# zhengyk19/vit-rpe-rope

Measured on AMD Instinct MI355X. Metric: train images/sec, CIFAR-10 ViT d=192 L=6 H=6, higher is better.
Workload: dtype bf16; 1 GPU; CIFAR-10-shaped 32x32 patch4 ViT d=192 L=6 H=6, --pos_encoding rope-axial theta=100, bf16, full train step (fwd+CE+bwd+AdamW), random-init weights; per_gpu_batch=512, global_batch=512, parallelism=dp1, hip_graph=True

## Files before the change

### include/vitpe_debug.h

```cpp
#ifndef VITPE_DEBUG_H
#define VITPE_DEBUG_H
#include "vitpe.h"
#ifdef __cplusplus
extern "C" {
#endif

int vitpe_selftest_mma(int dtype, const void* A, const void* Bt, const void* Brow, float* C_row,
                       float* C_tr, vitpe_stream_t stream);

int vitpe_debug_attn_occupancy(int which);
int vitpe_debug_wgrad_census(int dtype, const vitpe_wgrad_problem* problems, int nprob, unsigned long long* census,
                             vitpe_stream_t stream);
int vitpe_debug_attn_census(const void* xn, const void* wqkv, void* out, const float* cos, const float* sin,
                            int B, unsigned long long* census, vitpe_stream_t stream);
int vitpe_debug_attn32_census(const void* xn, const void* wqkv_wide, void* out, const float* cos, const float* sin,
                              int B, unsigned long long* census, int exp, vitpe_stream_t stream);
int vitpe_debug_tail2_census(const void* attn_out, const void* x_in, const void* Wp_packed, const float* bp,
                             const float* gamma, const float* beta, void* x_mid, float* mean2, float* rstd2,
                             void* xn_out, const void* W1_packed, const float* b1, const void* W2_packed,
                             const float* b2, void* gp_out, void* h_out, void* out, float* mean_out, float* rstd_out,
                             int M, int HID, unsigned long long* census, int exp, vitpe_stream_t stream);
int vitpe_debug_set_gemm2d_mt(int mt);
int vitpe_debug_set_wgrad_wide(int on);
int vitpe_debug_read_bw(const void* src, long long bytes, int depth, int workgroups, unsigned* sink, vitpe_stream_t stream);
#ifdef __cplusplus
}
#endif
#endif
```

### vit-rpe-rope_amd/csrc/attn.hip

```cpp
#include "attn_common.h"
#include <stdlib.h>
#include <type_traits>

namespace vitpe {

template <typename T, typename C, int KM, int NTH = 384>
VITPE_DEV void stage_tokens(const AttnArgs& a, int b, T* xs, T* hbuf, int hbuf_elems, float* s_tab, float* s_coef,
                            int tid, int nthreads, bool stage_tables) {
  constexpr int CHN = CH<T>::n;
  constexpr int DCH = C::LDX / CHN;
  constexpr int D = C::DD;
  const int N = C::ntok(a);
  const T* xg = reinterpret_cast<const T*>(a.xn) + (size_t)b * N * D;
  const Chunk16 zero = {0u, 0u, 0u, 0u};
  constexpr int TOTAL = C::NP * DCH;
  constexpr int ITERS = (TOTAL + NTH - 1) / NTH;
  Chunk16 v[ITERS];
#pragma unroll
  for (int it = 0; it < ITERS; ++it) {
    const int q = tid + it * nthreads, row = q / DCH, cc = q % DCH;
    v[it] = zero;
    if (q < TOTAL && row < N && cc * CHN < D) v[it] = *reinterpret_cast<const Chunk16*>(xg + (size_t)row * D + cc * CHN);
  }
  if (a.ln_gamma != nullptr) {
// ... 340 lines not shown
    f32x4 o[NT];
#pragma unroll
    for (int dt = 0; dt < NT; ++dt) o[dt] = z4;
#pragma unroll
    for (int sc = 0; sc < SC; ++sc) {
      const Frag<T> bp = acc_to_frag<T>(s[2 * sc], (2 * sc + 1 < MT) ? s[(2 * sc + 1 < MT) ? 2 * sc + 1 : 0] : z4);
#pragma unroll
      for (int dt = 0; dt < NT; ++dt) mma(vf[dt][sc], bp, o[dt]);
    }
    const float inv = __builtin_amdgcn_rcpf(l);
    if (sizeof(T) == 2) {
#pragma unroll
      for (int dp = 0; dp < NT; dp += 2) {
        uint32_t lo[2], hi[2];
#pragma unroll
        for (int w2 = 0; w2 < 2; ++w2) {
          bf16x2 pa, pb;
          const f32x4 oa = o[dp] * inv, ob = o[dp + 1] * inv;
          pa[0] = (bf16)oa[2 * w2]; pa[1] = (bf16)oa[2 * w2 + 1];
          pb[0] = (bf16)ob[2 * w2]; pb[1] = (bf16)ob[2 * w2 + 1];
          const auto r = __builtin_amdgcn_permlane16_swap(__builtin_bit_cast(uint32_t, pa), __builtin_bit_cast(uint32_t, pb),
                                                         false, false);
          lo[w2] = r[0]; hi[w2] = r[1];
        }
        const int f0 = 16 * (dp + (g & 1)) + 8 * (g >> 1);
        if (it < MT - 1 || i < N)
          *reinterpret_cast<Chunk16*>(outp + (size_t)i * D + f0) = (Chunk16){lo[0], lo[1], hi[0], hi[1]};
      }
    } else if (it < MT - 1 || i < N) {
#pragma unroll
      for (int dt = 0; dt < NT; ++dt)
        st4(outp + (size_t)i * D + 16 * dt + 4 * g, o[dt][0] * inv, o[dt][1] * inv, o[dt][2] * inv, o[dt][3] * inv);
    }
  }
  stamp(6);
}

template <typename T, typename C, int NTH>
VITPE_DEV void stage_rows_plain(const T* src, T* dst, int ld, int N, int tid) {
  constexpr int CHN = CH<T>::n, D = C::DD, CPRW = D / CHN, RPP = NTH / CPRW, ITERS = C::NP / RPP;
  const int cc = tid % CPRW, r0 = tid / CPRW;
  const Chunk16 zero = {0u, 0u, 0u, 0u};
  Chunk16 v[ITERS];
#pragma unroll
  for (int it = 0; it < ITERS; ++it) {
    const int row = r0 + it * RPP;
    v[it] = *reinterpret_cast<const Chunk16*>(src + (size_t)min(row, N - 1) * D + cc * CHN);
    if (row >= N) v[it] = zero;
  }
#pragma unroll
  for (int it = 0; it < ITERS; ++it) *reinterpret_cast<Chunk16*>(dst + (r0 + it * RPP) * ld + cc * CHN) = v[it];
}

template <int HD, int D, int MT, int KM, int NTOK, int IPW, bool LNF, bool MIXED, int PDEG = 7>
__global__ __launch_bounds__(64 * (D / HD) * IPW, 3) void attn_bwd_reg_kernel(AttnArgs a) {
  using T = bf16;
  using C = AttnCfg<T, HD, D, MT, 1, NTOK>;
  constexpr int NT = C::NT, KS = C::KS, HC = C::HC, SC = C::SC, NTH = 64 * C::H;
  static_assert(NT == 2 && HC == 1, "head dimension 32");
  constexpr int CSLD = HD / 2 + 8;
  constexpr int FRAG = 64 * 8;
  constexpr int XS_ELEMS = IPW * C::NP * C::LDX, DOS_ELEMS = IPW * C::H * MT * FRAG;
  __shared__ __attribute__((aligned(16))) T xs_all[XS_ELEMS > DOS_ELEMS ? XS_ELEMS : DOS_ELEMS];
  __shared__ __attribute__((aligned(16))) T qs_all[IPW * C::H * MT * FRAG];
  __shared__ __attribute__((aligned(16))) float s_tab[KM == KM_RELATIVE ? C::H * C::TABLD : 4];
  __shared__ __attribute__((aligned(16))) float s_coef[KM == KM_POLY ? C::PESZ : 4];
  __shared__ __attribute__((aligned(16))) float s_cos[KM == KM_ROPE ? C::NP * CSLD : 4];
  __shared__ __attribute__((aligned(16))) float s_sin[KM == KM_ROPE ? C::NP * CSLD : 4];
  __shared__ __attribute__((aligned(16))) float s_stat[IPW * C::H * 2 * C::NP];
  __shared__ float s_dtab[KM == KM_RELATIVE ? C::H * C::TABLD : 4];
  __shared__ float s_dcoef[C::H * (C::MAXDEG + 1)];
  __shared__ float s_dfreq[2 * C::H * (HD / 2)];

  const int N = C::ntok(a), P = N - 1;
  const int lane = threadIdx.x & 63;
  const int wave_all = __builtin_amdgcn_readfirstlane(threadIdx.x >> 6);
  const int img = wave_all / C::H, h = wave_all % C::H;
  const int b_raw = blockIdx.x * IPW + img;
  const bool live = b_raw < a.B;
  const int b = live ? b_raw : a.B - 1;
  const int tid_img = threadIdx.x % NTH;
  T* const xs = xs_all + img * C::NP * C::LDX;
  T* const qsw = qs_all + wave_all * MT * FRAG + lane * 8;
  T* const dsw = xs_all + wave_all * MT * FRAG + lane * 8;
  float* const lse_w = s_stat + (img * C::H + h) * 2 * C::NP;
  float* const del_w = lse_w + C::NP;
  float* const dtab_i = s_dtab;
  float* const dcoef_i = s_dcoef;
  float* const dfreq_i = s_dfreq;
  const int c = lane & 15, g = lane >> 4;
  const f32x4 z4 = {0.f, 0.f, 0.f, 0.f};
  constexpr bool mixed = (KM == KM_ROPE) && MIXED;

  const T* const Wh = reinterpret_cast<const T*>(a.wqkv) + ((size_t)h * 3 * NT * KS * 64 + lane) * 8;
  auto wload = [&](Frag<T> (&w)[NT][KS], int mat) {
#pragma unroll
    for (int nt = 0; nt < NT; ++nt)
#pragma unroll
      for (int ks = 0; ks < KS; ++ks) w[nt][ks] = ld_frag(Wh + (size_t)((mat * NT + nt) * KS + ks) * 64 * 8);
  };
  Frag<T> w[NT][KS];
  wload(w, 2);
  stage_tokens_fwd<T, C, KM, NTH, LNF>(a, b, xs, s_tab, s_coef, tid_img, false, IPW == 1 || img == 0);
  if (KM == KM_ROPE && !mixed) {
    constexpr int F4 = HD / 8;
    for (int q = threadIdx.x; q < C::NP * F4; q += NTH * IPW) {
      const int f4 = q % F4, row = q / F4;
      f32x4 cv = {1.f, 1.f, 1.f, 1.f}, sv = {0.f, 0.f, 0.f, 0.f};
      if (row >= 1 && row < N) {
        cv = *reinterpret_cast<const f32x4*>(a.cos + (size_t)(row - 1) * (HD / 2) + 4 * f4);
        sv = *reinterpret_cast<const f32x4*>(a.sin + (size_t)(row - 1) * (HD / 2) + 4 * f4);
      }
      *reinterpret_cast<f32x4*>(&s_cos[row * CSLD + 4 * f4]) = cv;
      *reinterpret_cast<f32x4*>(&s_sin[row * CSLD + 4 * f4]) = sv;
    }
  }
  if (KM == KM_RELATIVE)
    for (int q = threadIdx.x; q < C::H * C::TABLD; q += NTH * IPW) s_dtab[q] = 0.f;
  for (int q = threadIdx.x; q < C::H * (C::MAXDEG + 1); q += NTH * IPW) s_dcoef[q] = 0.f;
  for (int q = threadIdx.x; q < 2 * C::H * (HD / 2); q += NTH * IPW) s_dfreq[q] = 0.f;
  __syncthreads();

  const T* const xrow = xs + c * C::LDX + 8 * g;
  const unsigned hoff = mixed ? (unsigned)(h * P * (HD / 2)) : 0u;
  auto cs_vec = [&](int tok, int f, f32x4& cv, f32x4& sv) {
    if (!mixed) {
      cv = *reinterpret_cast<const f32x4*>(&s_cos[tok * CSLD + f]);
      sv = *reinterpret_cast<const f32x4*>(&s_sin[tok * CSLD + f]);
    } else {
      const bool ok = tok >= 1 && tok < N;
      const unsigned o = hoff + (unsigned)((min(max(tok, 1), N - 1) - 1) * (HD / 2) + f);
      const f32x4 cg = *reinterpret_cast<const f32x4*>(a.cos + o), sg = *reinterpret_cast<const f32x4*>(a.sin + o);
      cv = ok ? cg : (f32x4){1.f, 1.f, 1.f, 1.f};
      sv = ok ? sg : z4;
    }
  };
  auto proj_sw = [&](int tt, bool rope, float sc, Frag<T>& dst) {
    Frag<T> xf[KS];
#pragma unroll
    for (int ks = 0; ks < KS; ++ks) xf[ks] = ld_frag(xrow + 16 * tt * C::LDX + 32 * ks);
    __builtin_amdgcn_sched_barrier(0);
    f32x4 acc[NT] = {z4, z4};
#pragma unroll
    for (int ks = 0; ks < KS; ++ks)
#pragma unroll
      for (int nt = 0; nt < NT; ++nt) mma(w[nt][ks], xf[ks], acc[nt]);
    __builtin_amdgcn_sched_barrier(0);
    if (KM == KM_ROPE && rope) {
      f32x4 cv, sv;
      cs_vec(16 * tt + c, 4 * g, cv, sv);
      const f32x4 x1 = acc[0], x2 = acc[1];
      acc[0] = x1 * cv - x2 * sv;
      acc[1] = x1 * sv + x2 * cv;
    }
    dst = acc_to_frag<T>(acc[0] * sc, acc[1] * sc);
    asm volatile("" : "+v"(dst.v));
  };
  Frag<T> e0, e1;
#pragma unroll
  for (int t = 0; t < 8; ++t) {
    e0.v[t] = (bf16)((t < 4 && 4 * g + t == c) ? 1.0f : 0.0f);
    e1.v[t] = (bf16)((t >= 4 && 4 * g + t - 4 == c) ? 1.0f : 0.0f);
  }
  auto transpose_pair = [&](const Frag<T>& fa, const Frag<T>* fb, Frag<T>& d0, Frag<T>& d1) {
    f32x4 a0 = z4, a1 = z4, b0 = z4, b1 = z4;
    mma(fa, e0, a0);
    mma(fa, e1, a1);
    if (fb != nullptr) { mma(*fb, e0, b0); mma(*fb, e1, b1); }
    d0 = acc_to_frag<T>(a0, b0);
    d1 = acc_to_frag<T>(a1, b1);
  };

  const float qsc = a.scale * LOG2E;
  Frag<T> vkf[MT], kf[MT];
#pragma unroll
  for (int tt = 0; tt < MT; ++tt) proj_sw(tt, false, 1.0f, vkf[tt]);
  wload(w, 1);
  __builtin_amdgcn_sched_barrier(0);
#pragma unroll
  for (int tt = 0; tt < MT; ++tt) proj_sw(tt, true, 1.0f, kf[tt]);
  wload(w, 0);
  __builtin_amdgcn_sched_barrier(0);
#pragma unroll
  for (int tt = 0; tt < MT; ++tt) {
    Frag<T> qf;
    proj_sw(tt, true, qsc, qf);
    *reinterpret_cast<bf16x8*>(qsw + tt * FRAG) = qf.v;
  }
  __syncthreads();
  if (!live) return;
  {
    const T* dog = reinterpret_cast<const T*>(a.dout) + (size_t)b * N * D + h * HD;
    Frag<T> df[MT];
#pragma unroll
    for (int tt = 0; tt < MT; ++tt) {
      const int tok = 16 * tt + c;
      bf16x4 lo = {(bf16)0.f, (bf16)0.f, (bf16)0.f, (bf16)0.f}, hi = lo;
      if (tok < N) {
        lo = *reinterpret_cast<const bf16x4*>(dog + (size_t)tok * D + 4 * g);
        hi = *reinterpret_cast<const bf16x4*>(dog + (size_t)tok * D + 16 + 4 * g);
      }
      df[tt].v = __builtin_shufflevector(lo, hi, 0, 1, 2, 3, 4, 5, 6, 7);
    }
#pragma unroll
    for (int tt = 0; tt < MT; ++tt) *reinterpret_cast<bf16x8*>(dsw + tt * FRAG) = df[tt].v;
  }
  auto qf_load = [&](int tt) { Frag<T> f; f.v = *reinterpret_cast<const bf16x8*>(qsw + tt * FRAG); return f; };
  auto dof_load = [&](int tt) { Frag<T> f; f.v = *reinterpret_cast<const bf16x8*>(dsw + tt * FRAG); return f; };
  Frag<T> ktf[NT][SC];
#pragma unroll
  for (int scx = 0; scx < SC; ++scx)
    transpose_pair(kf[2 * scx], (2 * scx + 1 < MT) ? &kf[(2 * scx + 1 < MT) ? 2 * scx + 1 : 0] : nullptr, ktf[0][scx], ktf[1][scx]);

  T* const dqg = reinterpret_cast<T*>(a.out) + (size_t)b * N * 3 * D + h * HD;
  auto store_pair = [&](T* rowp, const f32x4& o0, const f32x4& o1, bool ok) {
    uint32_t lo[2], hi[2];
#pragma unroll
    for (int w2 = 0; w2 < 2; ++w2) {
      bf16x2 pa, pb;
      pa[0] = (bf16)o0[2 * w2]; pa[1] = (bf16)o0[2 * w2 + 1];
      pb[0] = (bf16)o1[2 * w2]; pb[1] = (bf16)o1[2 * w2 + 1];
      const auto r = __builtin_amdgcn_permlane16_swap(__builtin_bit_cast(uint32_t, pa), __builtin_bit_cast(uint32_t, pb), false, false);
      lo[w2] = r[0]; hi[w2] = r[1];
    }
    const int f0 = 16 * (g & 1) + 8 * (g >> 1);
    if (ok) *reinterpret_cast<Chunk16*>(rowp + f0) = (Chunk16){lo[0], lo[1], hi[0], hi[1]};
  };

  float cacc[PDEG + 1];
#pragma unroll
  for (int k = 0; k <= PDEG; ++k) cacc[k] = 0.f;
#pragma unroll
  for (int it = 0; it < MT; ++it) {
    __builtin_amdgcn_sched_barrier(0);
    const int i = 16 * it + c;
    const Frag<T> dof = dof_load(it), qfi = qf_load(it);
    f32x4 s[MT], dp[MT];
    float m = -1e30f;
    typedef __attribute__((ext_vector_type(4))) unsigned u32x4;
    const unsigned xyi = (KM == KM_POLY) ? reinterpret_cast<const unsigned*>(s_coef + C::H * C::PBLD)[i] : 0u;
    const float* const ptab = s_coef + (a.coeff_per_head ? h : 0) * C::PBLD;
    const bool qcls = (it == 0) && (c == 0);
#pragma unroll
    for (int jt = 0; jt < MT; ++jt) {
      s[jt] = z4;
      mma(kf[jt], qfi, s[jt]);
      dp[jt] = z4;
      mma(vkf[jt], dof, dp[jt]);
      const u32x4 xyj = (KM == KM_POLY) ? *reinterpret_cast<const u32x4*>(s_coef + C::H * C::PBLD + 16 * jt + 4 * g) : (u32x4){0u, 0u, 0u, 0u};
#pragma unroll
      for (int r = 0; r < 4; ++r) {
        const int j = 16 * jt + 4 * g + r;
        float v = s[jt][r];
        if (KM == KM_RELATIVE) v += pe_bias2<C, KM>(a, s_tab, s_coef, h, i, j, N);
        if (KM == KM_POLY) {
          const float bv = ptab[__builtin_amdgcn_sad_u8(xyi, xyj[r], 0u)];
          const bool cls = qcls || (jt == 0 && r == 0 && g == 0);
          v += cls ? 0.f : bv;
        }
        if (jt == MT - 1) v = (j < N) ? v : -1e30f;
        s[jt][r] = v;
        m = fmaxf(m, v);
      }
    }
    m = xg_max(m);
    float l = 0.f;
#pragma unroll
    for (int jt = 0; jt < MT; ++jt)
#pragma unroll
      for (int r = 0; r < 4; ++r) { const float p = __builtin_amdgcn_exp2f(s[jt][r] - m); s[jt][r] = p; l += p; }
    l = xg_sum(l);
    const float inv = __builtin_amdgcn_rcpf(l);
    float dl = 0.f;
#pragma unroll
    for (int jt = 0; jt < MT; ++jt)
#pragma unroll
      for (int r = 0; r < 4; ++r) { s[jt][r] *= inv; dl += s[jt][r] * dp[jt][r]; }
    dl = xg_sum(dl);
    if (g == 0) { lse_w[i] = m + __builtin_amdgcn_logf(l); del_w[i] = dl; }
    const bool qvalid = (it < MT - 1) || (i < N);
    float tacc[PDEG + 1];
#pragma unroll
    for (int k = 0; k <= PDEG; ++k) tacc[k] = 0.f;
#pragma unroll
    for (int jt = 0; jt < MT; ++jt) {
      if (KM == KM_POLY) __builtin_amdgcn_sched_barrier(0);
      const u32x4 xyj = (KM == KM_POLY) ? *reinterpret_cast<const u32x4*>(s_coef + C::H * C::PBLD + 16 * jt + 4 * g) : (u32x4){0u, 0u, 0u, 0u};
#pragma unroll
      for (int r = 0; r < 4; ++r) {
        const int j = 16 * jt + 4 * g + r;
        const bool valid = qvalid && ((jt < MT - 1) || (j < N));
        const float ds = valid ? s[jt][r] * (dp[jt][r] - dl) : 0.f;
        dp[jt][r] = ds;
        if (KM == KM_POLY) {
          const float dsk = (jt == 0 && r == 0) ? (g == 0 ? 0.f : ds) : ds;
          const float x = (float)__builtin_amdgcn_sad_u8(xyi, xyj[r], 0u);
          float pw = x;
          tacc[0] += dsk;
#pragma unroll
          for (int k = 1; k <= PDEG; ++k) { tacc[k] = fmaf(dsk, pw, tacc[k]); if (k < PDEG) pw *= x; }
        }
      }
    }
    if (KM == KM_POLY) {
      const float qm = (it == 0 && c == 0) ? 0.f : 1.f;
#pragma unroll
      for (int k = 0; k <= PDEG; ++k) {
        cacc[k] = fmaf(qm, tacc[k], cacc[k]);
        asm volatile("" : "+v"(cacc[k]));
      }
    }
    if (KM == KM_RELATIVE) {
#pragma unroll
      for (int jt = 0; jt < MT; ++jt) {
        float d0, d1;
        tile_diag_sums(dp[jt], lane, d0, d1);
        const int idx0 = 16 * (it - jt) + c + N - 1;
        if (g == 0) {
          if (idx0 >= 0 && idx0 <= 2 * N - 2) atomicAdd(&dtab_i[h * C::TABLD + idx0], d0);
          if (c >= 1 && idx0 - 16 >= 0 && idx0 - 16 <= 2 * N - 2) atomicAdd(&dtab_i[h * C::TABLD + idx0 - 16], d1);
        }
      }
    }
    f32x4 dqa[NT] = {z4, z4};
#pragma unroll
    for (int scx = 0; scx < SC; ++scx) {
      const Frag<T> bs = acc_to_frag<T>(dp[2 * scx], (2 * scx + 1 < MT) ? dp[(2 * scx + 1 < MT) ? 2 * scx + 1 : 0] : z4);
#pragma unroll
      for (int dt = 0; dt < NT; ++dt) mma(ktf[dt][scx], bs, dqa[dt]);
    }
    if (mixed) {
      const bool tok_ok = i >= 1 && i < N;
      f32x4 dph;
#pragma unroll
      for (int r = 0; r < 4; ++r) dph[r] = dqa[1][r] * (float)qfi.v[r] - dqa[0][r] * (float)qfi.v[4 + r];
      mixed_freq_grad_tile(dfreq_i, dph, i, tok_ok, 16 * it, h, C::H, P, a.grid, HD / 2, 4 * g, LN2, lane);
    }
    if (KM == KM_ROPE) {
      f32x4 cv, sv;
      cs_vec(min(i, C::NP - 1), 4 * g, cv, sv);
      const f32x4 d1 = dqa[0], d2 = dqa[1];
      dqa[0] = d1 * cv + d2 * sv;
      dqa[1] = d2 * cv - d1 * sv;
    }
    store_pair(dqg + (size_t)i * 3 * D, dqa[0] * a.scale, dqa[1] * a.scale, qvalid);
  }

  if (KM == KM_POLY) {
#pragma unroll
    for (int k = 0; k <= PDEG; ++k)
      if (k <= a.degree) {
        const float t = wave_sum(cacc[k]);
        if (lane == 0) atomicAdd(&dcoef_i[(a.coeff_per_head ? h : 0) * (C::MAXDEG + 1) + k], t);
      }
  }
  Frag<T> qtf[NT][SC], dotf[NT][SC];
  __builtin_amdgcn_sched_barrier(0);
#pragma unroll
  for (int scx = 0; scx < SC; ++scx) {
    const bool two = 2 * scx + 1 < MT;
    const Frag<T> qa = qf_load(2 * scx), qb = qf_load(two ? 2 * scx + 1 : 0);
    transpose_pair(qa, two ? &qb : nullptr, qtf[0][scx], qtf[1][scx]);
    const Frag<T> da = dof_load(2 * scx), db = dof_load(two ? 2 * scx + 1 : 0);
    transpose_pair(da, two ? &db : nullptr, dotf[0][scx], dotf[1][scx]);
  }
  __builtin_amdgcn_s_waitcnt(0xC07F);

#pragma unroll
  for (int jt = 0; jt < MT; ++jt) {
    __builtin_amdgcn_sched_barrier(0);
    const int j = 16 * jt + c;
    const bool kvalid = (jt < MT - 1) || (j < N);
    const unsigned xyk = (KM == KM_POLY) ? reinterpret_cast<const unsigned*>(s_coef + C::H * C::PBLD)[j] : 0u;
    const float* const ptab2 = s_coef + (a.coeff_per_head ? h : 0) * C::PBLD;
    const bool kcls = (jt == 0) && (c == 0);
    f32x4 p[MT], ds[MT];
#pragma unroll
    for (int it = 0; it < MT; ++it) {
      const Frag<T> dof = dof_load(it), qfi = qf_load(it);
      p[it] = z4;
      mma(qfi, kf[jt], p[it]);
      ds[it] = z4;
      mma(dof, vkf[jt], ds[it]);
      const f32x4 lse = *reinterpret_cast<const f32x4*>(&lse_w[16 * it + 4 * g]);
      const f32x4 dlv = *reinterpret_cast<const f32x4*>(&del_w[16 * it + 4 * g]);
      typedef __attribute__((ext_vector_type(4))) unsigned u32x4;
      const u32x4 xyq = (KM == KM_POLY) ? *reinterpret_cast<const u32x4*>(s_coef + C::H * C::PBLD + 16 * it + 4 * g) : (u32x4){0u, 0u, 0u, 0u};
#pragma unroll
      for (int r = 0; r < 4; ++r) {
        const int i = 16 * it + 4 * g + r;
        float sv = p[it][r];
        if (KM == KM_RELATIVE) sv += pe_bias2<C, KM>(a, s_tab, s_coef, h, i, j, N);
        if (KM == KM_POLY) {
          const float bv = ptab2[__builtin_amdgcn_sad_u8(xyk, xyq[r], 0u)];
          const bool cls = kcls || (it == 0 && r == 0 && g == 0);
          sv += cls ? 0.f : bv;
        }
        const bool valid = kvalid && ((it < MT - 1) || (i < N));
        const float pv = valid ? __builtin_amdgcn_exp2f(sv - lse[r]) : 0.f;
        p[it][r] = pv;
        ds[it][r] = pv * (ds[it][r] - dlv[r]);
      }
    }
    f32x4 dva[NT] = {z4, z4}, dka[NT] = {z4, z4};
#pragma unroll
    for (int scx = 0; scx < SC; ++scx) {
      const bool two = (2 * scx + 1 < MT);
      const Frag<T> bp = acc_to_frag<T>(p[2 * scx], two ? p[two ? 2 * scx + 1 : 0] : z4);
      const Frag<T> bs = acc_to_frag<T>(ds[2 * scx], two ? ds[two ? 2 * scx + 1 : 0] : z4);
#pragma unroll
      for (int dt = 0; dt < NT; ++dt) {
        mma(dotf[dt][scx], bp, dva[dt]);
        mma(qtf[dt][scx], bs, dka[dt]);
      }
    }
    dka[0] *= LN2; dka[1] *= LN2;
    if (mixed) {
      const bool tok_ok = j >= 1 && j < N;
      f32x4 dph;
#pragma unroll
      for (int r = 0; r < 4; ++r) dph[r] = dka[1][r] * (float)kf[jt].v[r] - dka[0][r] * (float)kf[jt].v[4 + r];
      mixed_freq_grad_tile(dfreq_i, dph, j, tok_ok, 16 * jt, h, C::H, P, a.grid, HD / 2, 4 * g, 1.0f, lane);
    }
    if (KM == KM_ROPE) {
      f32x4 cv, sv;
      cs_vec(min(j, C::NP - 1), 4 * g, cv, sv);
      const f32x4 d1 = dka[0], d2 = dka[1];
      dka[0] = d1 * cv + d2 * sv;
      dka[1] = d2 * cv - d1 * sv;
    }
    store_pair(dqg + (size_t)j * 3 * D + D, dka[0], dka[1], kvalid);
    store_pair(dqg + (size_t)j * 3 * D + 2 * D, dva[0], dva[1], kvalid);
  }

  __syncthreads();
  const int nrun = NTH * min(IPW, a.B - (int)blockIdx.x * IPW);
  if (KM == KM_RELATIVE) {
    for (int q = threadIdx.x; q < C::H * (2 * N - 1); q += nrun) {
      const int hh = q / (2 * N - 1), i = q % (2 * N - 1);
      atomicAdd(a.dtable + q, s_dtab[hh * C::TABLD + i]);
    }
  } else if (KM == KM_POLY) {
    const int nh = a.coeff_per_head ? C::H : 1;
    for (int q = threadIdx.x; q < nh * (a.degree + 1); q += nrun) {
      const int hh = q / (a.degree + 1), k = q % (a.degree + 1);
      atomicAdd(a.dcoeff + q, s_dcoef[hh * (C::MAXDEG + 1) + k]);
    }
  } else if (mixed) {
    for (int q = threadIdx.x; q < 2 * C::H * (HD / 2); q += nrun) atomicAdd(a.dfreqs + q, s_dfreq[q]);
  }
}

template <typename T, int HD, int D, int MT, int HPP, int KM, int NTOK>
__global__ __launch_bounds__(384) void attn_bwd_kernel(AttnArgs a) {
  using C = AttnCfg<T, HD, D, MT, HPP, NTOK>;
  __shared__ __attribute__((aligned(16))) T xs[C::NP * C::LDX];
  __shared__ __attribute__((aligned(16))) T hb[4 * HPP * C::HSZ];
  __shared__ __attribute__((aligned(16))) float s_tab[KM == KM_RELATIVE ? C::H * C::TABLD : 4];
  __shared__ __attribute__((aligned(16))) float s_coef[KM == KM_POLY ? C::PESZ : 4];
  __shared__ __attribute__((aligned(16))) float s_stat[HPP * 2 * C::NP];
  __shared__ float s_dtab[KM == KM_RELATIVE ? C::H * C::TABLD : 4];
  __shared__ float s_dcoef[C::H * (C::MAXDEG + 1)];
  __shared__ float s_dfreq[2 * C::H * (HD / 2)];
  constexpr int SLD = HPP * HD + Pad<T>::elems;
  __shared__ __attribute__((aligned(16))) T s_dq[3 * C::NP * SLD];

  const int N = C::ntok(a);
  const int b = blockIdx.x;
  const int lane = threadIdx.x & 63;
  const int wave = __builtin_amdgcn_readfirstlane(threadIdx.x >> 6);
  const int c = lane & 15, g = lane >> 4;
  const int P = N - 1;
  WFrags<T, C> wf;
  {
    const int hh = wave / 3, mat = wave % 3;
    if (hh < HPP && hh < C::H) load_w<T, C>(a, wf, hh, mat, lane);
  }
  stage_tokens<T, C, KM>(a, b, xs, hb, 4 * HPP * C::HSZ, s_tab, s_coef, threadIdx.x, 384, true);
  if (KM == KM_RELATIVE)
    for (int q = threadIdx.x; q < C::H * C::TABLD; q += 384) s_dtab[q] = 0.f;
  for (int q = threadIdx.x; q < C::H * (C::MAXDEG + 1); q += 384) s_dcoef[q] = 0.f;
  for (int q = threadIdx.x; q < 2 * C::H * (HD / 2); q += 384) s_dfreq[q] = 0.f;
  __syncthreads();

  constexpr int CHN = CH<T>::n;
  const T* dog = reinterpret_cast<const T*>(a.dout) + (size_t)b * N * D;
  T* dq = reinterpret_cast<T*>(a.out) + (size_t)b * N * 3 * D;
  const bool mixed = (KM == KM_ROPE) && a.mode == PE_ROPE_MIXED;
  const f32x4 z4 = {0.f, 0.f, 0.f, 0.f};

  for (int h0 = 0; h0 < C::H; h0 += HPP) {
    {
      const int hh = wave / 3, mat = wave % 3, h = h0 + hh;
      if (hh < HPP && h < C::H) project_head<T, C, KM>(a, wf, xs, hb + (mat * HPP + hh) * C::HSZ, h, mat, lane);
      if (hh < HPP && h + HPP < C::H) load_w<T, C>(a, wf, h + HPP, mat, lane);
    }
    for (int q = threadIdx.x; q < HPP * N * (HD / CHN); q += 384) {
      const int hh = q / (N * (HD / CHN)), rem = q % (N * (HD / CHN));
      const int row = rem / (HD / CHN), cc = rem % (HD / CHN);
      if (h0 + hh < C::H)
        *reinterpret_cast<Chunk16*>(hb + (3 * HPP + hh) * C::HSZ + row * C::LDH + cc * CHN) =
            *reinterpret_cast<const Chunk16*>(dog + (size_t)row * D + (h0 + hh) * HD + cc * CHN);
// ... 324 lines not shown
    if (a.ln_gamma != nullptr) hipLaunchKernelGGL((attn_fwd_kernel<T, HD, D, MT, KM, NTOK, IPW, true>), grid, block, 0, s, a);
    else hipLaunchKernelGGL((attn_fwd_kernel<T, HD, D, MT, KM, NTOK, IPW, false>), grid, block, 0, s, a);
  }
  VITPE_CHECK_LAUNCH();
}

template <typename T, int HD, int D, int MT, int HPP, int NTOK>
static int launch_attn2(bool bwd, const AttnArgs& a, hipStream_t s) {
  switch (a.mode) {
    case PE_RELATIVE: return launch_attn3<T, HD, D, MT, HPP, KM_RELATIVE, NTOK>(bwd, a, s);
    case PE_POLY: return launch_attn3<T, HD, D, MT, HPP, KM_POLY, NTOK>(bwd, a, s);
    case PE_ROPE_AXIAL:
    case PE_ROPE_MIXED: return launch_attn3<T, HD, D, MT, HPP, KM_ROPE, NTOK>(bwd, a, s);
    default: return launch_attn3<T, HD, D, MT, HPP, KM_PLAIN, NTOK>(bwd, a, s);
  }
}

template <typename T, int HD, int D, int MT, int HPP>
static int launch_attn(bool bwd, const AttnArgs& a, hipStream_t s) {
  if (a.N == 65) return launch_attn2<T, HD, D, MT, HPP, 65>(bwd, a, s);
  return launch_attn2<T, HD, D, MT, HPP, 0>(bwd, a, s);
}

static int dispatch_attn(bool bwd, int dtype, int D, int HD, const AttnArgs& a, hipStream_t s) {
  const int MT = (a.N + 15) / 16;
  if (HD != 32 || MT != 5) return (int)hipErrorNotSupported;
  if (dtype == 1) {
    if (D == 192) return launch_attn<bf16, 32, 192, 5, 2>(bwd, a, s);
    if (D == 96) return launch_attn<bf16, 32, 96, 5, 2>(bwd, a, s);
  } else if (dtype == 0) {
    if (D == 192) return launch_attn<float, 32, 192, 5, 1>(bwd, a, s);
    if (D == 96) return launch_attn<float, 32, 96, 5, 1>(bwd, a, s);
  }
  return (int)hipErrorNotSupported;
}

extern "C" int vitpe_fused_attention_supported(int dtype, int N, int D, int HD) {
  const int MT = (N + 15) / 16;
  return (dtype == 0 || dtype == 1) && HD == 32 && MT == 5 && (D == 192 || D == 96);
}

static int fused_fwd(int dtype, const void* x, const float* gamma, const float* beta, const float* mean,
                     const float* rstd, void* xn_out, const void* wqkv, void* out, int B, int N, int D, int HD,
                     const PeArgs& pe, hipStream_t stream) {
  VITPE_REQUIRE(x && wqkv && out && B >= 0 && N >= 2);
  VITPE_REQUIRE(pe_ok(pe, N, 0, 0));
  if (B == 0) return 0;
  AttnArgs a = attn_args(pe, B, N, 0, HD);
  a.xn = x; a.wqkv = wqkv; a.out = out;
  a.ln_gamma = gamma; a.ln_beta = beta; a.ln_mean = mean; a.ln_rstd = rstd; a.xn_out = xn_out;
  return dispatch_attn(false, dtype, D, HD, a, stream);
}

static int fused_bwd(int dtype, const void* x, const float* gamma, const float* beta, const float* mean,
                     const float* rstd, const void* wqkv, const void* dout, void* dqkv, int B, int N, int D, int HD,
                     const PeArgs& pe, float* dtable, float* dcoeff, float* dfreqs, hipStream_t stream) {
  VITPE_REQUIRE(x && wqkv && dout && dqkv && B >= 0 && N >= 2);
  VITPE_REQUIRE(pe_ok(pe, N, 0, 0));
  VITPE_REQUIRE(pe_grads_ok(pe.mode, dtable, dcoeff, dfreqs));
  if (B == 0) return 0;
  AttnArgs a = attn_args(pe, B, N, 0, HD);
  a.xn = x; a.wqkv = wqkv; a.out = dqkv; a.dout = dout;
  a.dtable = dtable; a.dcoeff = dcoeff; a.dfreqs = dfreqs;
  a.ln_gamma = gamma; a.ln_beta = beta; a.ln_mean = mean; a.ln_rstd = rstd;
  return dispatch_attn(true, dtype, D, HD, a, stream);
}

extern "C" int vitpe_fused_attention_fwd(int dtype, const void* xn, const void* wqkv, void* out, int B, int N,
                                         int D, int HD, int mode, const float* cos, const float* sin,
                                         const float* table, const float* coeff, int grid, int degree,
                                         int coeff_per_head, hipStream_t stream) {
  return fused_fwd(dtype, xn, nullptr, nullptr, nullptr, nullptr, nullptr, wqkv, out, B, N, D, HD,
                   {mode, cos, sin, table, coeff, grid, degree, coeff_per_head}, stream);
}

extern "C" int vitpe_fused_attention_fwd_ln(int dtype, const void* x, const float* gamma, const float* beta,
                                            const float* mean, const float* rstd, void* xn_out, const void* wqkv,
                                            void* out, int B, int N, int D, int HD, int mode, const float* cos,
                                            const float* sin, const float* table, const float* coeff, int grid,
                                            int degree, int coeff_per_head, hipStream_t stream) {
  VITPE_REQUIRE(gamma && beta && mean && rstd);
  return fused_fwd(dtype, x, gamma, beta, mean, rstd, xn_out, wqkv, out, B, N, D, HD,
                   {mode, cos, sin, table, coeff, grid, degree, coeff_per_head}, stream);
}

extern "C" int vitpe_fused_attention_bwd(int dtype, const void* xn, const void* wqkv, const void* dout,
                                         void* dqkv, int B, int N, int D, int HD, int mode, const float* cos,
                                         const float* sin, const float* table, const float* coeff, int grid,
                                         int degree, int coeff_per_head, float* dtable, float* dcoeff,
                                         float* dfreqs, hipStream_t stream) {
  return fused_bwd(dtype, xn, nullptr, nullptr, nullptr, nullptr, wqkv, dout, dqkv, B, N, D, HD,
                   {mode, cos, sin, table, coeff, grid, degree, coeff_per_head}, dtable, dcoeff, dfreqs, stream);
}

extern "C" int vitpe_fused_attention_bwd_ln(int dtype, const void* x, const float* gamma, const float* beta,
                                            const float* mean, const float* rstd, const void* wqkv, const void* dout,
                                            void* dqkv, int B, int N, int D, int HD, int mode, const float* cos,
                                            const float* sin, const float* table, const float* coeff, int grid,
                                            int degree, int coeff_per_head, float* dtable, float* dcoeff,
                                            float* dfreqs, hipStream_t stream) {
  VITPE_REQUIRE(gamma && beta && mean && rstd);
  return fused_bwd(dtype, x, gamma, beta, mean, rstd, wqkv, dout, dqkv, B, N, D, HD,
                   {mode, cos, sin, table, coeff, grid, degree, coeff_per_head}, dtable, dcoeff, dfreqs, stream);
}

extern "C" int vitpe_debug_attn_census(const void* xn, const void* wqkv, void* out, const float* cos, const float* sin,
                                       int B, unsigned long long* census, hipStream_t stream) {
  VITPE_REQUIRE(xn && wqkv && out && cos && sin && census && B > 0);
  AttnArgs a = attn_args({PE_ROPE_AXIAL, cos, sin, nullptr, nullptr, 8, 0, 0}, B, 65, 0, 32);
  a.xn = xn; a.wqkv = wqkv; a.out = out; a.census = census;
  hipLaunchKernelGGL((attn_fwd_kernel<bf16, 32, 192, 5, KM_ROPE, 65, 2, false, true>), dim3((B + 1) / 2), dim3(768), 0, stream, a);
  VITPE_CHECK_LAUNCH();
}

extern "C" int vitpe_debug_attn_occupancy(int which) {
  int n = -1;
  hipError_t e;
  if (which == 0)
    e = hipOccupancyMaxActiveBlocksPerMultiprocessor(&n, attn_fwd_kernel<bf16, 32, 192, 5, KM_ROPE, 65, 2, true>, 768, 0);
  else if (which == 1)
    e = hipOccupancyMaxActiveBlocksPerMultiprocessor(&n, attn_fwd_kernel<bf16, 32, 192, 5, KM_PLAIN, 65, 2, true>, 768, 0);
  else
    e = hipOccupancyMaxActiveBlocksPerMultiprocessor(&n, attn_bwd_reg_kernel<32, 192, 5, KM_ROPE, 65, 2, true, false>, 768, 0);
  return e == hipSuccess ? n : -(int)e;
}
```

### vit-rpe-rope_amd/csrc/attn_common.h

```cpp
#pragma once
#include "common.h"

namespace vitpe {

struct AttnArgs {
  const void* xn;
  const void* wqkv;
  void* out;
  const void* dout;
  const float* cos;
  const float* sin;
  const float* table;
  const float* coeff;
  float* dtable;
  float* dcoeff;
  float* dfreqs;
  const void* qkv;
  int B, N, H;
  int mode, grid, degree, coeff_per_head;
  float scale;
  const float* ln_gamma;
  const float* ln_beta;
  const float* ln_mean;
  const float* ln_rstd;
  void* xn_out;
  unsigned long long* census;
  void* qkv_out;
  float* tab_slab;
  const unsigned long long* rng;
  unsigned drop_thr;
  float drop_rs;
  int cls_only;
};

struct PeArgs {
  int mode;
  const float *cos, *sin, *table, *coeff;
  int grid, degree, coeff_per_head;
};

inline bool pe_ok(const PeArgs& pe, int N, int H, int hmax) {
  if (pe.mode == PE_ROPE_AXIAL || pe.mode == PE_ROPE_MIXED) {
    if (!pe.cos || !pe.sin || pe.grid * pe.grid != N - 1) return false;
    if (pe.mode == PE_ROPE_MIXED && hmax && H > hmax) return false;
  }
  if (pe.mode == PE_RELATIVE && !pe.table) return false;
  if (pe.mode == PE_POLY && (!pe.coeff || pe.degree < 0 || pe.degree > 7 || pe.grid * pe.grid != N - 1)) return false;
  return pe.mode >= PE_NONE && pe.mode <= PE_ROPE_MIXED;
}

inline bool pe_grads_ok(int mode, const float* dtable, const float* dcoeff, const float* dfreqs) {
  if (mode == PE_RELATIVE) return dtable != nullptr;
  if (mode == PE_POLY) return dcoeff != nullptr;
  if (mode == PE_ROPE_MIXED) return dfreqs != nullptr;
  return true;
}

inline AttnArgs attn_args(const PeArgs& pe, int B, int N, int H, int HD) {
  AttnArgs a{};
  a.cos = pe.cos; a.sin = pe.sin; a.table = pe.table; a.coeff = pe.coeff;
  a.mode = pe.mode; a.grid = pe.grid; a.degree = pe.degree; a.coeff_per_head = pe.coeff_per_head;
  a.B = B; a.N = N; a.H = H;
  a.scale = 1.0f / sqrtf((float)HD);
  return a;
}

constexpr float LOG2E = 1.4426950408889634f;
constexpr float LN2 = 0.6931471805599453f;

enum { KM_PLAIN = 0, KM_RELATIVE = 1, KM_POLY = 2, KM_ROPE = 3, KM_ROPE_TABLES = 4 };

template <typename T, int HD, int D, int MT, int HPP, int NTOK>
struct AttnCfg {
  static constexpr int H = D / HD;
  static constexpr int NT = HD / 16;
  static constexpr int KS = D / 32;
  static constexpr int HC = HD / 32;
  static constexpr int NP = 16 * MT;
  static constexpr int SC = (MT + 1) / 2;
  static constexpr int VR = 32 * SC;
  static constexpr int LDX = D + (sizeof(T) == 2 ? 2 : 1) * Pad<T>::elems;
  static constexpr int LDH = HD + (sizeof(T) == 2 ? 2 : 1) * Pad<T>::elems;
  static constexpr int HSZ = VR * LDH;
  static constexpr int QSZ = NP * LDH;
  static constexpr int TABLD = 2 * NP;
// ... 133 lines not shown
```

Baseline: 359,900 images/sec.

## Skip attention-backward query tiles whose output gradient is entirely zero

The attention backward kernel now checks, per 16-token query tile, whether the incoming output gradient is all zero using a wave ballot. Zero tiles skip the score/softmax recompute and the dK/dV contributions, and their dQ rows are written as zeros; a dense specialization is kept for the case where every tile is nonzero. This targets layers such as the last block under CLS-only classification, where only the CLS row carries gradient. It also masks padded lanes in the final odd tile out of the exp/softmax work, privatizes the poly/mixed-rope gradient accumulators per wave instead of using shared atomics, and adds optional timestamp census instrumentation plus a debug switch. The extra cost is a ballot per tile, more code paths, and more shared memory for the privatized accumulators.

After: 360,700 images/sec (median of 6 runs). Within noise of the previous version (+0.2%).

```diff
diff --git a/include/vitpe_debug.h b/include/vitpe_debug.h
--- a/include/vitpe_debug.h
+++ b/include/vitpe_debug.h
@@ -15,6 +15,8 @@
                             int B, unsigned long long* census, vitpe_stream_t stream);
 int vitpe_debug_attn32_census(const void* xn, const void* wqkv_wide, void* out, const float* cos, const float* sin,
                               int B, unsigned long long* census, int exp, vitpe_stream_t stream);
+int vitpe_debug_attn_bwd_census(const void* xn, const void* wqkv, const void* dout, void* dqkv, const float* cos,
+                                const float* sin, int B, unsigned long long* census, vitpe_stream_t stream);
 int vitpe_debug_tail2_census(const void* attn_out, const void* x_in, const void* Wp_packed, const float* bp,
                              const float* gamma, const float* beta, void* x_mid, float* mean2, float* rstd2,
                              void* xn_out, const void* W1_packed, const float* b1, const void* W2_packed,
@@ -22,6 +24,7 @@
                              int M, int HID, unsigned long long* census, int exp, vitpe_stream_t stream);
 int vitpe_debug_set_gemm2d_mt(int mt);
 int vitpe_debug_set_wgrad_wide(int on);
+int vitpe_debug_set_attn_bwd_skip(int on);
 int vitpe_debug_read_bw(const void* src, long long bytes, int depth, int workgroups, unsigned* sink, vitpe_stream_t stream);
 #ifdef __cplusplus
 }
diff --git a/vit-rpe-rope_amd/csrc/attn.hip b/vit-rpe-rope_amd/csrc/attn.hip
--- a/vit-rpe-rope_amd/csrc/attn.hip
+++ b/vit-rpe-rope_amd/csrc/attn.hip
@@ -416,7 +416,9 @@
   for (int it = 0; it < ITERS; ++it) *reinterpret_cast<Chunk16*>(dst + (r0 + it * RPP) * ld + cc * CHN) = v[it];
 }
 
-template <int HD, int D, int MT, int KM, int NTOK, int IPW, bool LNF, bool MIXED, int PDEG = 7>
+template <bool V> struct BoolTag { static constexpr bool value = V; };
+
+template <int HD, int D, int MT, int KM, int NTOK, int IPW, bool LNF, bool MIXED, int PDEG = 7, bool CENSUS = false>
 __global__ __launch_bounds__(64 * (D / HD) * IPW, 3) void attn_bwd_reg_kernel(AttnArgs a) {
   using T = bf16;
   using C = AttnCfg<T, HD, D, MT, 1, NTOK>;
@@ -432,9 +434,10 @@
   __shared__ __attribute__((aligned(16))) float s_cos[KM == KM_ROPE ? C::NP * CSLD : 4];
   __shared__ __attribute__((aligned(16))) float s_sin[KM == KM_ROPE ? C::NP * CSLD : 4];
   __shared__ __attribute__((aligned(16))) float s_stat[IPW * C::H * 2 * C::NP];
-  __shared__ float s_dtab[KM == KM_RELATIVE ? C::H * C::TABLD : 4];
-  __shared__ float s_dcoef[C::H * (C::MAXDEG + 1)];
-  __shared__ float s_dfreq[2 * C::H * (HD / 2)];
+  constexpr int DTAB_N = C::H * C::TABLD, DCOEF_N = C::MAXDEG + 1, DFREQ_N = 2 * C::H * (HD / 2), NWAVE = IPW * C::H;
+  __shared__ float s_dtab[KM == KM_RELATIVE ? IPW * DTAB_N : 4];
+  __shared__ float s_dcoef[KM == KM_POLY ? NWAVE * DCOEF_N : 4];
+  __shared__ float s_dfreq[(KM == KM_ROPE && MIXED) ? NWAVE * DFREQ_N : 4];
 
   const int N = C::ntok(a), P = N - 1;
   const int lane = threadIdx.x & 63;
@@ -449,12 +452,20 @@
   T* const dsw = xs_all + wave_all * MT * FRAG + lane * 8;
   float* const lse_w = s_stat + (img * C::H + h) * 2 * C::NP;
   float* const del_w = lse_w + C::NP;
-  float* const dtab_i = s_dtab;
-  float* const dcoef_i = s_dcoef;
-  float* const dfreq_i = s_dfreq;
+  float* const dtab_i = s_dtab + (KM == KM_RELATIVE ? img * DTAB_N : 0);
+  float* const dcoef_i = s_dcoef + (KM == KM_POLY ? wave_all * DCOEF_N : 0);
+  float* const dfreq_i = s_dfreq + ((KM == KM_ROPE && MIXED) ? wave_all * DFREQ_N : 0);
   const int c = lane & 15, g = lane >> 4;
   const f32x4 z4 = {0.f, 0.f, 0.f, 0.f};
   constexpr bool mixed = (KM == KM_ROPE) && MIXED;
+  auto stamp = [&](int slot) {
+    if (CENSUS) {
+      __builtin_amdgcn_sched_barrier(0);
+      if (lane == 0) a.census[((size_t)blockIdx.x * 16 + wave_all) * 16 + slot] = __builtin_amdgcn_s_memtime();
+      __builtin_amdgcn_sched_barrier(0);
+    }
+  };
+  stamp(0);
 
   const T* const Wh = reinterpret_cast<const T*>(a.wqkv) + ((size_t)h * 3 * NT * KS * 64 + lane) * 8;
   auto wload = [&](Frag<T> (&w)[NT][KS], int mat) {
@@ -480,10 +491,14 @@
     }
   }
   if (KM == KM_RELATIVE)
-    for (int q = threadIdx.x; q < C::H * C::TABLD; q += NTH * IPW) s_dtab[q] = 0.f;
-  for (int q = threadIdx.x; q < C::H * (C::MAXDEG + 1); q += NTH * IPW) s_dcoef[q] = 0.f;
-  for (int q = threadIdx.x; q < 2 * C::H * (HD / 2); q += NTH * IPW) s_dfreq[q] = 0.f;
+    for (int q = threadIdx.x; q < IPW * DTAB_N; q += NTH * IPW) s_dtab[q] = 0.f;
+  if (KM == KM_POLY)
+    for (int q = threadIdx.x; q < NWAVE * DCOEF_N; q += NTH * IPW) s_dcoef[q] = 0.f;
+  if (KM == KM_ROPE && MIXED)
+    for (int q = threadIdx.x; q < NWAVE * DFREQ_N; q += NTH * IPW) s_dfreq[q] = 0.f;
+  stamp(1);
   __syncthreads();
+  stamp(2);
 
   const T* const xrow = xs + c * C::LDX + 8 * g;
   const unsigned hoff = mixed ? (unsigned)(h * P * (HD / 2)) : 0u;
@@ -551,11 +566,15 @@
     proj_sw(tt, true, qsc, qf);
     *reinterpret_cast<bf16x8*>(qsw + tt * FRAG) = qf.v;
   }
+  stamp(3);
   __syncthreads();
+  stamp(4);
   if (!live) return;
+  constexpr bool ODD = NTOK == 16 * (MT - 1) + 1;
+  unsigned nz = 0u;
+  Frag<T> df[MT];
   {
     const T* dog = reinterpret_cast<const T*>(a.dout) + (size_t)b * N * D + h * HD;
-    Frag<T> df[MT];
 #pragma unroll
     for (int tt = 0; tt < MT; ++tt) {
       const int tok = 16 * tt + c;
@@ -569,12 +588,21 @@
 #pragma unroll
     for (int tt = 0; tt < MT; ++tt) *reinterpret_cast<bf16x8*>(dsw + tt * FRAG) = df[tt].v;
   }
+  auto tile_nz = [&](int tt) { return ((nz >> tt) & 1u) != 0u; };
   auto qf_load = [&](int tt) { Frag<T> f; f.v = *reinterpret_cast<const bf16x8*>(qsw + tt * FRAG); return f; };
   auto dof_load = [&](int tt) { Frag<T> f; f.v = *reinterpret_cast<const bf16x8*>(dsw + tt * FRAG); return f; };
   Frag<T> ktf[NT][SC];
 #pragma unroll
   for (int scx = 0; scx < SC; ++scx)
     transpose_pair(kf[2 * scx], (2 * scx + 1 < MT) ? &kf[(2 * scx + 1 < MT) ? 2 * scx + 1 : 0] : nullptr, ktf[0][scx], ktf[1][scx]);
+#pragma unroll
+  for (int tt = 0; tt < MT; ++tt) {
+    typedef __attribute__((ext_vector_type(4))) unsigned u32x4;
+    const u32x4 bits = __builtin_bit_cast(u32x4, df[tt].v);
+    if (__builtin_amdgcn_ballot_w64(((bits[0] | bits[1]) | (bits[2] | bits[3])) != 0u) != 0ull) nz |= 1u << tt;
+  }
+  if (a.bwd_dense) nz = (1u << MT) - 1u;
+  nz = __builtin_amdgcn_readfirstlane(nz);
 
   T* const dqg = reinterpret_cast<T*>(a.out) + (size_t)b * N * 3 * D + h * HD;
   auto store_pair = [&](T* rowp, const f32x4& o0, const f32x4& o1, bool ok) {
@@ -594,10 +622,16 @@
   float cacc[PDEG + 1];
 #pragma unroll
   for (int k = 0; k <= PDEG; ++k) cacc[k] = 0.f;
+  stamp(5);
 #pragma unroll
   for (int it = 0; it < MT; ++it) {
     __builtin_amdgcn_sched_barrier(0);
     const int i = 16 * it + c;
+    if (!tile_nz(it)) {
+      if ((it < MT - 1) || (i < N))
+        *reinterpret_cast<Chunk16*>(dqg + (size_t)i * 3 * D + 16 * (g & 1) + 8 * (g >> 1)) = (Chunk16){0u, 0u, 0u, 0u};
+      continue;
+    }
     const Frag<T> dof = dof_load(it), qfi = qf_load(it);
     f32x4 s[MT], dp[MT];
     float m = -1e30f;
@@ -615,6 +649,7 @@
 #pragma unroll
       for (int r = 0; r < 4; ++r) {
         const int j = 16 * jt + 4 * g + r;
+        if (ODD && jt == MT - 1 && r > 0) { s[jt][r] = 0.f; continue; }
         float v = s[jt][r];
         if (KM == KM_RELATIVE) v += pe_bias2<C, KM>(a, s_tab, s_coef, h, i, j, N);
         if (KM == KM_POLY) {
@@ -632,14 +667,23 @@
 #pragma unroll
     for (int jt = 0; jt < MT; ++jt)
 #pragma unroll
-      for (int r = 0; r < 4; ++r) { const float p = __builtin_amdgcn_exp2f(s[jt][r] - m); s[jt][r] = p; l += p; }
+      for (int r = 0; r < 4; ++r) {
+        if (ODD && jt == MT - 1 && r > 0) continue;
+        const float p = __builtin_amdgcn_exp2f(s[jt][r] - m);
+        s[jt][r] = p;
+        l += p;
+      }
     l = xg_sum(l);
     const float inv = __builtin_amdgcn_rcpf(l);
     float dl = 0.f;
 #pragma unroll
     for (int jt = 0; jt < MT; ++jt)
 #pragma unroll
-      for (int r = 0; r < 4; ++r) { s[jt][r] *= inv; dl += s[jt][r] * dp[jt][r]; }
+      for (int r = 0; r < 4; ++r) {
+        if (ODD && jt == MT - 1 && r > 0) continue;
+        s[jt][r] *= inv;
+        dl += s[jt][r] * dp[jt][r];
+      }
     dl = xg_sum(dl);
     if (g == 0) { lse_w[i] = m + __builtin_amdgcn_logf(l); del_w[i] = dl; }
     const bool qvalid = (it < MT - 1) || (i < N);
@@ -653,6 +697,7 @@
 #pragma unroll
       for (int r = 0; r < 4; ++r) {
         const int j = 16 * jt + 4 * g + r;
+        if (ODD && jt == MT - 1 && r > 0) { dp[jt][r] = 0.f; continue; }
         const bool valid = qvalid && ((jt < MT - 1) || (j < N));
         const float ds = valid ? s[jt][r] * (dp[jt][r] - dl) : 0.f;
         dp[jt][r] = ds;
@@ -715,103 +760,143 @@
     for (int k = 0; k <= PDEG; ++k)
       if (k <= a.degree) {
         const float t = wave_sum(cacc[k]);
-        if (lane == 0) atomicAdd(&dcoef_i[(a.coeff_per_head ? h : 0) * (C::MAXDEG + 1) + k], t);
-      }
-  }
-  Frag<T> qtf[NT][SC], dotf[NT][SC];
-  __builtin_amdgcn_sched_barrier(0);
-#pragma unroll
-  for (int scx = 0; scx < SC; ++scx) {
-    const bool two = 2 * scx + 1 < MT;
-    const Frag<T> qa = qf_load(2 * scx), qb = qf_load(two ? 2 * scx + 1 : 0);
-    transpose_pair(qa, two ? &qb : nullptr, qtf[0][scx], qtf[1][scx]);
-    const Frag<T> da = dof_load(2 * scx), db = dof_load(two ? 2 * scx + 1 : 0);
-    transpose_pair(da, two ? &db : nullptr, dotf[0][scx], dotf[1][scx]);
-  }
-  __builtin_amdgcn_s_waitcnt(0xC07F);
-
-#pragma unroll
-  for (int jt = 0; jt < MT; ++jt) {
+        if (lane == 0) dcoef_i[k] = t;
+      }
+  }
+  stamp(6);
+  auto step2 = [&](auto dense_tag) {
+    constexpr bool DENSE = decltype(dense_tag)::value;
+    Frag<T> qtf[NT][SC], dotf[NT][SC];
     __builtin_amdgcn_sched_barrier(0);
-    const int j = 16 * jt + c;
-    const bool kvalid = (jt < MT - 1) || (j < N);
-    const unsigned xyk = (KM == KM_POLY) ? reinterpret_cast<const unsigned*>(s_coef + C::H * C::PBLD)[j] : 0u;
-    const float* const ptab2 = s_coef + (a.coeff_per_head ? h : 0) * C::PBLD;
-    const bool kcls = (jt == 0) && (c == 0);
-    f32x4 p[MT], ds[MT];
-#pragma unroll
-    for (int it = 0; it < MT; ++it) {
-      const Frag<T> dof = dof_load(it), qfi = qf_load(it);
-      p[it] = z4;
-      mma(qfi, kf[jt], p[it]);
-      ds[it] = z4;
-      mma(dof, vkf[jt], ds[it]);
-      const f32x4 lse = *reinterpret_cast<const f32x4*>(&lse_w[16 * it + 4 * g]);
-      const f32x4 dlv = *reinterpret_cast<const f32x4*>(&del_w[16 * it + 4 * g]);
-      typedef __attribute__((ext_vector_type(4))) unsigned u32x4;
-      const u32x4 xyq = (KM == KM_POLY) ? *reinterpret_cast<const u32x4*>(s_coef + C::H * C::PBLD + 16 * it + 4 * g) : (u32x4){0u, 0u, 0u, 0u};
-#pragma unroll
-      for (int r = 0; r < 4; ++r) {
-        const int i = 16 * it + 4 * g + r;
-        float sv = p[it][r];
-        if (KM == KM_RELATIVE) sv += pe_bias2<C, KM>(a, s_tab, s_coef, h, i, j, N);
-        if (KM == KM_POLY) {
-          const float bv = ptab2[__builtin_amdgcn_sad_u8(xyk, xyq[r], 0u)];
-          const bool cls = kcls || (it == 0 && r == 0 && g == 0);
-          sv += cls ? 0.f : bv;
-        }
-        const bool valid = kvalid && ((it < MT - 1) || (i < N));
-        const float pv = valid ? __builtin_amdgcn_exp2f(sv - lse[r]) : 0.f;
-        p[it][r] = pv;
-        ds[it][r] = pv * (ds[it][r] - dlv[r]);
-      }
-    }
-    f32x4 dva[NT] = {z4, z4}, dka[NT] = {z4, z4};
-#pragma unroll
+  #pragma unroll
     for (int scx = 0; scx < SC; ++scx) {
-      const bool two = (2 * scx + 1 < MT);
-      const Frag<T> bp = acc_to_frag<T>(p[2 * scx], two ? p[two ? 2 * scx + 1 : 0] : z4);
-      const Frag<T> bs = acc_to_frag<T>(ds[2 * scx], two ? ds[two ? 2 * scx + 1 : 0] : z4);
-#pragma unroll
-      for (int dt = 0; dt < NT; ++dt) {
-        mma(dotf[dt][scx], bp, dva[dt]);
-        mma(qtf[dt][scx], bs, dka[dt]);
-      }
-    }
-    dka[0] *= LN2; dka[1] *= LN2;
-    if (mixed) {
-      const bool tok_ok = j >= 1 && j < N;
-      f32x4 dph;
-#pragma unroll
-      for (int r = 0; r < 4; ++r) dph[r] = dka[1][r] * (float)kf[jt].v[r] - dka[0][r] * (float)kf[jt].v[4 + r];
-      mixed_freq_grad_tile(dfreq_i, dph, j, tok_ok, 16 * jt, h, C::H, P, a.grid, HD / 2, 4 * g, 1.0f, lane);
-    }
-    if (KM == KM_ROPE) {
-      f32x4 cv, sv;
-      cs_vec(min(j, C::NP - 1), 4 * g, cv, sv);
-      const f32x4 d1 = dka[0], d2 = dka[1];
-      dka[0] = d1 * cv + d2 * sv;
-      dka[1] = d2 * cv - d1 * sv;
-    }
-    store_pair(dqg + (size_t)j * 3 * D + D, dka[0], dka[1], kvalid);
-    store_pair(dqg + (size_t)j * 3 * D + 2 * D, dva[0], dva[1], kvalid);
-  }
-
+      const bool two = 2 * scx + 1 < MT;
+      if (!DENSE && ((nz >> (2 * scx)) & 3u) == 0u) continue;
+      const Frag<T> qa = qf_load(2 * scx), qb = qf_load(two ? 2 * scx + 1 : 0);
+      transpose_pair(qa, two ? &qb : nullptr, qtf[0][scx], qtf[1][scx]);
+      const Frag<T> da = dof_load(2 * scx), db = dof_load(two ? 2 * scx + 1 : 0);
+      transpose_pair(da, two ? &db : nullptr, dotf[0][scx], dotf[1][scx]);
+    }
+    __builtin_amdgcn_s_waitcnt(0xC07F);
+    stamp(7);
+
+  #pragma unroll
+    for (int jt = 0; jt < MT; ++jt) {
+      __builtin_amdgcn_sched_barrier(0);
+      const int j = 16 * jt + c;
+      const bool kvalid = (jt < MT - 1) || (j < N);
+      const unsigned xyk = (KM == KM_POLY) ? reinterpret_cast<const unsigned*>(s_coef + C::H * C::PBLD)[j] : 0u;
+      const float* const ptab2 = s_coef + (a.coeff_per_head ? h : 0) * C::PBLD;
+      const bool kcls = (jt == 0) && (c == 0);
+      auto qtile = [&](int it, f32x4& pt, f32x4& dst) {
+        const Frag<T> dof = dof_load(it), qfi = qf_load(it);
+        mma(qfi, kf[jt], pt);
+        mma(dof, vkf[jt], dst);
+        const f32x4 lse = *reinterpret_cast<const f32x4*>(&lse_w[16 * it + 4 * g]);
+        const f32x4 dlv = *reinterpret_cast<const f32x4*>(&del_w[16 * it + 4 * g]);
+        typedef __attribute__((ext_vector_type(4))) unsigned u32x4;
+        const u32x4 xyq = (KM == KM_POLY) ? *reinterpret_cast<const u32x4*>(s_coef + C::H * C::PBLD + 16 * it + 4 * g) : (u32x4){0u, 0u, 0u, 0u};
+  #pragma unroll
+        for (int r = 0; r < 4; ++r) {
+          const int i = 16 * it + 4 * g + r;
+          if (ODD && it == MT - 1 && r > 0) { pt[r] = 0.f; dst[r] = 0.f; continue; }
+          float sv = pt[r];
+          if (KM == KM_RELATIVE) sv += pe_bias2<C, KM>(a, s_tab, s_coef, h, i, j, N);
+          if (KM == KM_POLY) {
+            const float bv = ptab2[__builtin_amdgcn_sad_u8(xyk, xyq[r], 0u)];
+            const bool cls = kcls || (it == 0 && r == 0 && g == 0);
+            sv += cls ? 0.f : bv;
+          }
+          const bool valid = kvalid && ((it < MT - 1) || (i < N));
+          const float pv = valid ? __builtin_amdgcn_exp2f(sv - lse[r]) : 0.f;
+          pt[r] = pv;
+          dst[r] = pv * (dst[r] - dlv[r]);
+        }
+      };
+      f32x4 dva[NT] = {z4, z4}, dka[NT] = {z4, z4};
+      if constexpr (DENSE) {
+        f32x4 p[MT], ds[MT];
+  #pragma unroll
+        for (int it = 0; it < MT; ++it) { p[it] = z4; ds[it] = z4; qtile(it, p[it], ds[it]); }
+  #pragma unroll
+        for (int scx = 0; scx < SC; ++scx) {
+          const bool two = (2 * scx + 1 < MT);
+          const Frag<T> bp = acc_to_frag<T>(p[2 * scx], two ? p[two ? 2 * scx + 1 : 0] : z4);
+          const Frag<T> bs = acc_to_frag<T>(ds[2 * scx], two ? ds[two ? 2 * scx + 1 : 0] : z4);
+  #pragma unroll
+          for (int dt = 0; dt < NT; ++dt) {
+            mma(dotf[dt][scx], bp, dva[dt]);
+            mma(qtf[dt][scx], bs, dka[dt]);
+          }
+        }
+      } else {
+  #pragma unroll
+        for (int scx = 0; scx < SC; ++scx) {
+          const bool two = (2 * scx + 1 < MT);
+          if (((nz >> (2 * scx)) & 3u) == 0u) continue;
+          f32x4 pa = z4, pb = z4, dsa = z4, dsb = z4;
+          if (tile_nz(2 * scx)) qtile(2 * scx, pa, dsa);
+          if (two && tile_nz(2 * scx + 1)) qtile(two ? 2 * scx + 1 : 0, pb, dsb);
+          const Frag<T> bp = acc_to_frag<T>(pa, pb);
+          const Frag<T> bs = acc_to_frag<T>(dsa, dsb);
+  #pragma unroll
+          for (int dt = 0; dt < NT; ++dt) {
+            mma(dotf[dt][scx], bp, dva[dt]);
+            mma(qtf[dt][scx], bs, dka[dt]);
+          }
+        }
+      }
+      dka[0] *= LN2; dka[1] *= LN2;
+      if (mixed) {
+        const bool tok_ok = j >= 1 && j < N;
+        f32x4 dph;
+  #pragma unroll
+        for (int r = 0; r < 4; ++r) dph[r] = dka[1][r] * (float)kf[jt].v[r] - dka[0][r] * (float)kf[jt].v[4 + r];
+        mixed_freq_grad_tile(dfreq_i, dph, j, tok_ok, 16 * jt, h, C::H, P, a.grid, HD / 2, 4 * g, 1.0f, lane);
+      }
+      if (KM == KM_ROPE) {
+        f32x4 cv, sv;
+        cs_vec(min(j, C::NP - 1), 4 * g, cv, sv);
+        const f32x4 d1 = dka[0], d2 = dka[1];
+        dka[0] = d1 * cv + d2 * sv;
+        dka[1] = d2 * cv - d1 * sv;
+      }
+      store_pair(dqg + (size_t)j * 3 * D + D, dka[0], dka[1], kvalid);
+      store_pair(dqg + (size_t)j * 3 * D + 2 * D, dva[0], dva[1], kvalid);
+    }
+
+  };
+  if constexpr (KM == KM_POLY) step2(BoolTag<false>{});
+  else if (nz == (1u << MT) - 1u) step2(BoolTag<true>{});
+  else step2(BoolTag<false>{});
+
+  stamp(8);
   __syncthreads();
   const int nrun = NTH * min(IPW, a.B - (int)blockIdx.x * IPW);
   if (KM == KM_RELATIVE) {
     for (int q = threadIdx.x; q < C::H * (2 * N - 1); q += nrun) {
       const int hh = q / (2 * N - 1), i = q % (2 * N - 1);
-      atomicAdd(a.dtable + q, s_dtab[hh * C::TABLD + i]);
+      float t = s_dtab[hh * C::TABLD + i];
+#pragma unroll
+      for (int im = 1; im < IPW; ++im) t += s_dtab[im * DTAB_N + hh * C::TABLD + i];
+      atomicAdd(a.dtable + q, t);
     }
   } else if (KM == KM_POLY) {
     const int nh = a.coeff_per_head ? C::H : 1;
     for (int q = threadIdx.x; q < nh * (a.degree + 1); q += nrun) {
       const int hh = q / (a.degree + 1), k = q % (a.degree + 1);
-      atomicAdd(a.dcoeff + q, s_dcoef[hh * (C::MAXDEG + 1) + k]);
+      float t = 0.f;
+      for (int wv = 0; wv < NWAVE; ++wv)
+        if (!a.coeff_per_head || wv % C::H == hh) t += s_dcoef[wv * DCOEF_N + k];
+      atomicAdd(a.dcoeff + q, t);
     }
   } else if (mixed) {
-    for (int q = threadIdx.x; q < 2 * C::H * (HD / 2); q += nrun) atomicAdd(a.dfreqs + q, s_dfreq[q]);
+    for (int q = threadIdx.x; q < DFREQ_N; q += nrun) {
+      float t = 0.f;
+#pragma unroll
+      for (int wv = 0; wv < NWAVE; ++wv) t += s_dfreq[wv * DFREQ_N + q];
+      atomicAdd(a.dfreqs + q, t);
+    }
   }
 }
 
@@ -1242,6 +1327,9 @@
   return dispatch_attn(false, dtype, D, HD, a, stream);
 }
 
+static bool g_bwd_skip = true;
+extern "C" int vitpe_debug_set_attn_bwd_skip(int on) { g_bwd_skip = on != 0; return 0; }
+
 static int fused_bwd(int dtype, const void* x, const float* gamma, const float* beta, const float* mean,
                      const float* rstd, const void* wqkv, const void* dout, void* dqkv, int B, int N, int D, int HD,
                      const PeArgs& pe, float* dtable, float* dcoeff, float* dfreqs, hipStream_t stream) {
@@ -1253,6 +1341,7 @@
   a.xn = x; a.wqkv = wqkv; a.out = dqkv; a.dout = dout;
   a.dtable = dtable; a.dcoeff = dcoeff; a.dfreqs = dfreqs;
   a.ln_gamma = gamma; a.ln_beta = beta; a.ln_mean = mean; a.ln_rstd = rstd;
+  a.bwd_dense = g_bwd_skip ? 0 : 1;
   return dispatch_attn(true, dtype, D, HD, a, stream);
 }
 
@@ -1300,6 +1389,16 @@
   AttnArgs a = attn_args({PE_ROPE_AXIAL, cos, sin, nullptr, nullptr, 8, 0, 0}, B, 65, 0, 32);
   a.xn = xn; a.wqkv = wqkv; a.out = out; a.census = census;
   hipLaunchKernelGGL((attn_fwd_kernel<bf16, 32, 192, 5, KM_ROPE, 65, 2, false, true>), dim3((B + 1) / 2), dim3(768), 0, stream, a);
+  VITPE_CHECK_LAUNCH();
+}
+
+extern "C" int vitpe_debug_attn_bwd_census(const void* xn, const void* wqkv, const void* dout, void* dqkv, const float* cos,
+                                           const float* sin, int B, unsigned long long* census, hipStream_t stream) {
+  VITPE_REQUIRE(xn && wqkv && dout && dqkv && cos && sin && census && B > 0);
+  AttnArgs a = attn_args({PE_ROPE_AXIAL, cos, sin, nullptr, nullptr, 8, 0, 0}, B, 65, 0, 32);
+  a.xn = xn; a.wqkv = wqkv; a.out = dqkv; a.dout = dout; a.census = census;
+  a.bwd_dense = g_bwd_skip ? 0 : 1;
+  hipLaunchKernelGGL((attn_bwd_reg_kernel<32, 192, 5, KM_ROPE, 65, 2, false, false, 7, true>), dim3((B + 1) / 2), dim3(768), 0, stream, a);
   VITPE_CHECK_LAUNCH();
 }
 
diff --git a/vit-rpe-rope_amd/csrc/attn_common.h b/vit-rpe-rope_amd/csrc/attn_common.h
--- a/vit-rpe-rope_amd/csrc/attn_common.h
+++ b/vit-rpe-rope_amd/csrc/attn_common.h
@@ -31,6 +31,7 @@
   unsigned drop_thr;
   float drop_rs;
   int cls_only;
+  int bwd_dense;
 };
 
 struct PeArgs {
```
